# drtconway/zotmer

Hardware: AMD Instinct MI355X
Metric: Gk-mers/sec kmerize k=25 on synthetic 150bp FASTQ; achieved HBM GB/s fraction (higher is better)
Workload: dtype u64

## Files before the change

### zotmer_amd/csrc/context.hip

```cpp
#include <stdarg.h>
#include <string.h>

#include "internal.hpp"
#include <vector>

namespace zk {

int fail(zk_ctx* c, int code, const char* fmt, ...) {
    char buf[512];
    va_list ap;
    va_start(ap, fmt);
    vsnprintf(buf, sizeof buf, fmt, ap);
    va_end(ap);
    if (c) c->last_error = buf;
    return code;
}

void arena_reset(zk_ctx* c) { c->arena_off = 0; }

int arena_alloc(zk_ctx* c, uint64_t bytes, void** p) {
    const uint64_t need = (bytes + 255) & ~255ull;
    if (c->arena_off + need > c->arena_size) {
        if (c->arena_off != 0)
            return fail(c, ZK_ENOMEM, "workspace too small: %llu bytes in use, %llu more needed, %llu reserved (call zk_reserve)",
// ... 202 lines not shown
    if (c->status) (void)hipFree(c->status);
    if (c->part16) (void)hipFree(c->part16);
    if (c->d_ticket) (void)hipFree(c->d_ticket);
    if (c->d_xticket) (void)hipFree(c->d_xticket);
    if (c->d_err) (void)hipFree(c->d_err);
    if (c->d_scalars) (void)hipFree(c->d_scalars);
    if (c->h_scalars) (void)hipHostFree(c->h_scalars);
    if (c->own_stream && c->stream) (void)hipStreamDestroy(c->stream);
    delete c;
}

const char* zk_last_error(zk_ctx* c) { return c ? c->last_error.c_str() : g_create_error.c_str(); }

int zk_set_stream(zk_ctx* c, void* hip_stream) {
    if (!c) return ZK_EINVAL;
    enter(c);
    ZK_HIP(c, hipStreamSynchronize(c->stream));
    if (c->own_stream) { (void)hipStreamDestroy(c->stream); c->own_stream = false; }
    if (hip_stream) c->stream = (hipStream_t)hip_stream;
    else {
        ZK_HIP(c, hipStreamCreateWithFlags(&c->stream, hipStreamNonBlocking));
        c->own_stream = true;
    }
    return ZK_OK;
}

void* zk_get_stream(zk_ctx* c) { return c ? (void*)c->stream : nullptr; }

int zk_sync(zk_ctx* c) {
    if (!c) return ZK_EINVAL;
    enter(c);
    ZK_HIP(c, hipStreamSynchronize(c->stream));
    return ZK_OK;
}

int zk_reserve(zk_ctx* c, uint64_t workspace_bytes) {
    if (!c) return ZK_EINVAL;
    enter(c);
    if (workspace_bytes <= c->arena_size) return ZK_OK;
    arena_reset(c);
    void* p;
    ZK_TRY(arena_alloc(c, workspace_bytes, &p));
    arena_reset(c);
    return ZK_OK;
}

int zk_release_workspace(zk_ctx* c) {
    if (!c) return ZK_EINVAL;
    enter(c);
    ZK_HIP(c, hipStreamSynchronize(c->stream));
    if (c->arena) { ZK_HIP(c, hipFree(c->arena)); c->arena = nullptr; c->arena_size = 0; c->arena_off = 0; }
    if (c->aux) { ZK_HIP(c, hipFree(c->aux)); c->aux = nullptr; c->aux_size = 0; }
    if (c->status) { ZK_HIP(c, hipFree(c->status)); c->status = nullptr; c->status_words = 0; c->epoch = 0; }
    if (c->part16) { ZK_HIP(c, hipFree(c->part16)); c->part16 = nullptr; c->part16_words = 0; }
    return ZK_OK;
}

int zk_mem_info(zk_ctx* c, uint64_t* free_bytes, uint64_t* total_bytes) {
    if (!c) return ZK_EINVAL;
    enter(c);
    size_t f = 0, t = 0;
    ZK_HIP(c, hipMemGetInfo(&f, &t));
    if (free_bytes) *free_bytes = f;
    if (total_bytes) *total_bytes = t;
    return ZK_OK;
}

int zk_tune(zk_ctx* c, int what, int value) {
    if (!c) return ZK_EINVAL;
    enter(c);
    if (what == ZK_TUNE_SORT_VARIANT) { c->sort_variant = value; return ZK_OK; }
    if (what == ZK_TUNE_PAIRS_VARIANT) { c->pairs_variant = value; return ZK_OK; }
    if (what == ZK_TUNE_SHORT_SORT) { c->short_sort = value; return ZK_OK; }
    if (what == ZK_TUNE_SIDE_DIV) { c->side_div = value; return ZK_OK; }
    if (what == ZK_TUNE_WIDE_TILES) { c->wide_tiles = value ? 1 : 0; return ZK_OK; }
    if (what == ZK_TUNE_PACKED_PAIRS) { c->packed_pairs = value ? 1 : 0; return ZK_OK; }
    if (what == ZK_TUNE_EARLY_COLLAPSE) { c->early_collapse = value < 0 ? 0 : (value > 3 ? 3 : value); return ZK_OK; }
    if (what == ZK_TUNE_COMM_SELF_LOOP) { c->comm_self_loop = value ? 1 : 0; return ZK_OK; }
    if (what == ZK_TUNE_COMM_CHUNK) { c->comm_chunk_bytes = value > 0 ? (uint64_t)value : 0; return ZK_OK; }
    if (what == ZK_TUNE_STREAM_PASS) {
#ifdef ZK_PHASES
        c->stream_pass = value < 0 ? 0 : value;
#else
        if (value < 0 || value > 3) return fail(c, ZK_EINVAL, "stream pass variant %d (0, 1 or 3)", value);
        c->stream_pass = value;
#endif
        return ZK_OK;
    }
    if (what == ZK_TUNE_TAG_WORDS) { c->tag_words = value < 0 ? 0 : (value > 2 ? 2 : value); return ZK_OK; }
    if (what == ZK_TUNE_DEDUPE_VARIANT) { c->dedupe_variant = value < 0 ? -1 : (value & 3); return ZK_OK; }
    if (what == ZK_TUNE_KWAY) { c->kway = value < 0 ? 0 : (value > 2 ? 2 : value); return ZK_OK; }
    if (what == ZK_TUNE_TILE_SORT) { c->tile_sort = value ? 1 : 0; return ZK_OK; }
    if (what == ZK_TUNE_TAG_PASS) { c->tag_pass = value ? 1 : 0; return ZK_OK; }
    if (what == ZK_TUNE_DEDUPE_BITS) { c->dedupe_bits = value < 0 ? 0 : value; return ZK_OK; }
    if (what == ZK_TUNE_DEDUPE_LIMIT) { c->dedupe_limit = value < 1 ? 1 : (value > 65536 ? 65536 : value); return ZK_OK; }
    if (what == ZK_TUNE_STREAM_RANGES) { c->stream_ranges = value < 0 ? 0 : (value > 4096 ? 4096 : value); return ZK_OK; }
    if (what == ZK_TUNE_XCD_GROUP) {
        if (value < 0 || value > 32 || (value & (value - 1))) return fail(c, ZK_EINVAL, "xcd group must be 0 or a power of two <= 32");
        c->xcd_group = value;
        return ZK_OK;
    }
    return fail(c, ZK_EINVAL, "unknown tuning knob %d", what);
}

int zk_debug_buffer(zk_ctx* c, void* d_buf) {
    if (!c) return ZK_EINVAL;
    enter(c);
    c->dbg = (u64*)d_buf;
    return ZK_OK;
}

int zk_profile(zk_ctx* c, int enable) {
    if (!c) return ZK_EINVAL;
    enter(c);
    ZK_HIP(c, hipStreamSynchronize(c->stream));
    for (auto& r : c->prof) { (void)hipEventDestroy(r.a); (void)hipEventDestroy(r.b); }
    c->prof.clear();
    c->profile = enable != 0;
    return ZK_OK;
}

int zk_profile_read(zk_ctx* c, int tag, uint64_t* launches, double* total_ms, uint64_t* total_bytes) {
    if (!c) return ZK_EINVAL;
    enter(c);
    ZK_HIP(c, hipStreamSynchronize(c->stream));
    uint64_t n = 0, bytes = 0;
    double ms = 0;
    for (auto& r : c->prof) {
        if (r.tag != tag) continue;
        float t = 0;
        ZK_HIP(c, hipEventElapsedTime(&t, r.a, r.b));
        n++; ms += t; bytes += r.bytes;
    }
    if (launches) *launches = n;
    if (total_ms) *total_ms = ms;
    if (total_bytes) *total_bytes = bytes;
    return ZK_OK;
}

int zk_alloc(zk_ctx* c, uint64_t bytes, void** dptr) {
    if (!c || !dptr) return ZK_EINVAL;
    enter(c);
    *dptr = nullptr;
    if (bytes == 0) bytes = 256;
    hipError_t e = hipMalloc(dptr, bytes);
    if (e != hipSuccess) return fail(c, ZK_ENOMEM, "hipMalloc(%llu) failed: %s", (unsigned long long)bytes, hipGetErrorString(e));
    return ZK_OK;
}

int zk_free(zk_ctx* c, void* dptr) {
    if (!c) return ZK_EINVAL;
    enter(c);
    if (dptr) { ZK_HIP(c, hipStreamSynchronize(c->stream)); ZK_HIP(c, hipFree(dptr)); }
    return ZK_OK;
}

int zk_host_alloc(zk_ctx* c, uint64_t bytes, void** ptr) {
    if (!c || !ptr) return ZK_EINVAL;
    enter(c);
    *ptr = nullptr;
    hipError_t e = hipHostMalloc(ptr, bytes ? bytes : 256, hipHostMallocDefault);
    if (e != hipSuccess) return fail(c, ZK_ENOMEM, "hipHostMalloc(%llu) failed: %s", (unsigned long long)bytes, hipGetErrorString(e));
    return ZK_OK;
}

int zk_host_free(zk_ctx* c, void* ptr) {
    if (!c) return ZK_EINVAL;
// ... 41 lines not shown
```

### zotmer_amd/csrc/internal.hpp

```cpp
#pragma once
#include <hip/hip_runtime.h>
#include <stdint.h>
#include <stdio.h>
#include <string>
#include <vector>

#include "../../include/zotk.h"
#include "common.hpp"

struct zk_ctx {
    int device = 0;
    hipStream_t stream = nullptr;
    bool own_stream = false;
    int num_cus = 256;
    int sort_variant = 3;
    int short_sort = 0;
    int packed_pairs = 1;
    int wide_tiles = 1;
    int early_collapse = 1;
    int side_div = 8;
    int pairs_variant = 7;
    int stream_pass = 1;
    int tag_words = 2;
    int dedupe_variant = 0;
// ... 36 lines not shown

    void* ring = nullptr;

    struct ProfRec { int tag; uint64_t bytes; hipEvent_t a, b; };
    bool profile = false;
    std::vector<ProfRec> prof;
};

namespace zk {

int fail(zk_ctx* c, int code, const char* fmt, ...);
static inline void enter(zk_ctx* c) {
    int d = -1;
    if (c && (hipGetDevice(&d) != hipSuccess || d != c->device)) (void)hipSetDevice(c->device);
}
#define ZK_HIP(c, call)                                                                         \
    do {                                                                                        \
        hipError_t e__ = (call);                                                                \
        if (e__ != hipSuccess)                                                                  \
            return zk::fail((c), ZK_EHIP, "%s failed: %s (%s:%d)", #call, hipGetErrorString(e__), __FILE__, __LINE__); \
    } while (0)
#define ZK_TRY(expr)             \
    do {                         \
        int r__ = (expr);        \
        if (r__ != ZK_OK) return r__; \
    } while (0)

void arena_reset(zk_ctx* c);
int arena_alloc(zk_ctx* c, uint64_t bytes, void** p);
int arena_require(zk_ctx* c, uint64_t want, uint64_t must);
int aux_require(zk_ctx* c, uint64_t bytes, char** p);
int lookback_begin(zk_ctx* c, uint64_t words, uint32_t tiles, u32* epoch, u32* ticket_base);
int part16_begin(zk_ctx* c, uint64_t words, unsigned short** out);
int check_device_error(zk_ctx* c);

void prof_begin(zk_ctx* c, int tag, uint64_t algorithmic_bytes);
void prof_end(zk_ctx* c);
void prof_add_bytes(zk_ctx* c, int tag, uint64_t bytes);

static inline uint64_t div_up(uint64_t a, uint64_t b) { return (a + b - 1) / b; }

constexpr int MAX_PASSES = 8;
struct PassPlan {
    int passes;
    int shift[MAX_PASSES];
    int bits[MAX_PASSES];
};
int sort_workspace_bytes(uint64_t n, bool pairs, uint64_t* bytes);
int sort_keys(zk_ctx* c, u64* keys, u64* alt, uint64_t n, int key_bits, u64** result);
int sort_pairs(zk_ctx* c, u64* keys, u64* alt, u32* vals, u32* valt, uint64_t n, int key_bits, u64** rk, u32** rv);
int sort_keys_upper(zk_ctx* c, u64* keys, u64* alt, uint64_t n, int key_bits, int lo_bit, u64** result, int prof_tag = ZK_PROF_PASS_PACKED);
int sort_pairs_upper(zk_ctx* c, u64* keys, u64* alt, u32* vals, u32* valt, uint64_t n, int key_bits, int lo_bit, u64** rk, u32** rv);
int sort_pairs_mirrored(zk_ctx* c, const u64* src_k, const u32* src_v, u64* keys, u64* alt, u32* vals, u32* valt, uint64_t n, int K,
                        u64** rk, u32** rv, int lo_bit = 0);
int sort_pairs_rbits(zk_ctx* c);
struct StreamSample { int shift; uint64_t value; double max_ratio; uint64_t seen = 0, distinct = 0; bool want_distinct = false; };
struct StreamTags { bool written = false; u64* cuts = nullptr; uint32_t blocks = 0; };
struct StreamSrc { const u8* stream; uint64_t n_bytes; int K; int mode; int lo_bit; int hi_bit = 0; StreamSample* sample = nullptr;
                   StreamTags* tags = nullptr; };
int sort_rbits(zk_ctx* c);
PassPlan sort_plan_upper(zk_ctx* c, int key_bits, int lo_bit);
struct MirrorHist { int passes; int shift[4]; int bits[4]; u64* raw; };
int sort_first_bits(zk_ctx* c, int key_bits, int lo_bit);
struct DedupeResult {
    uint64_t n_out = 0;
    uint32_t flags = 0;
    uint32_t n_big = 0;
    u64 *cuts = nullptr, *nwords = nullptr, *incl = nullptr, *big = nullptr, *work = nullptr;
    u32* sub = nullptr;
    uint32_t chunks = 0;
    int pack = 0;
};
int dedupe_pass(zk_ctx* c, const u64* keys, uint64_t n, int key_bits, int b, int pack, u64* work, uint64_t cap, DedupeResult* r,
                uint64_t* n_in = nullptr, uint64_t max_chunks = 0, const u32* tags = nullptr, const u64* tag_cuts = nullptr);
int expand_tags(zk_ctx* c, const u32* tags, const u64* cuts, uint32_t blocks, int tag_bits, u64* keys_out, uint64_t first_block = 0, uint64_t n_blocks = 0);
int dedupe_finish(zk_ctx* c, const DedupeResult& r, u64* out_k, u32* out_c, u64* out_m = nullptr, int K = 0, int gbases = 0,
                  u64** mirror_hist = nullptr, int* mirror_group_bits = nullptr, bool packed_out = false);
int sort_keys_upper_counted(zk_ctx* c, u64* keys, u64* alt, uint64_t n, int key_bits, int lo_bit, u64* counted, u64** result);
int collapse_pass(zk_ctx* c, const u64* keys, uint64_t n, int shift, int bits, int pack, u64* out, uint64_t cap, uint64_t* n_out,
                  uint64_t max_tiles = 0);
int sort_stream(zk_ctx* c, const StreamSrc& src, u64* buf_a, u64* buf_b, uint64_t cap, uint64_t* n_keys,
                uint64_t acgt[4], u64** result);
struct StreamRows { u32* rows = nullptr; u64* offs = nullptr; u32 ranges = 0, radix = 0; u32* gcodes = nullptr; u16* gvalid = nullptr;
                    u32 strands = 1; };
int stream_hist(zk_ctx* c, const u8* stream, uint64_t n_bytes, int K, int mode, const PassPlan& plan, u64* ghist, u32 gstride,
                u64* d_acgt, u64* d_n, u64* rec_info, u64* sample, u32 sample_cap, int sample_shift, u64 sample_value, u32* sample_n,
                void* image_room, uint64_t image_room_bytes, StreamRows* out);
struct StreamPlanes { u16* dig; int shift, bits; };
int stream_pass0(zk_ctx* c, uint64_t n_bytes, int K, int mode, int shift, int bits, const u64* ghist0, const StreamRows& rows,
                 uint64_t first_nl, bool uniform, u64* kout, uint64_t n, int variant, const StreamPlanes* planes = nullptr);
int stream_pass1(zk_ctx* c, const u32* tags, const u16* dig, uint64_t n, const u64* ghist0, uint32_t radix0, int bits1, u32* tout, u64* cuts);
int tile_sort_top_bits(uint64_t n, int key_bits, int rbits);
int tile_sort(zk_ctx* c, u64* keys, u32* vals, uint64_t n, int key_bits, int top, bool* declined);
int tile_sort_count(zk_ctx* c, const u64* keys, uint64_t n, int key_bits, int top, u64* uniq, u32* counts, uint64_t cap, uint64_t* n_unique,
                    bool* declined);
int trim(zk_ctx* c, const u64* keys, const void* cnts, int cbits, uint64_t n, u64 lo, u64 hi, u64* ok, void* oc,
         uint64_t cap, uint64_t* n_out);
int project_dedupe(zk_ctx* c, const u64* keys, uint64_t n, int shift, u64* out, uint64_t cap, uint64_t* n_out);
int subsample(zk_ctx* c, const u64* keys, uint64_t n, u64 seed, double p, u64* out, uint64_t cap, uint64_t* n_out);
int sample_pairs(zk_ctx* c, const u64* keys, const u64* cnts, uint64_t n, u64 seed, double p, u64* ok, u64* oc, uint64_t cap,
                 uint64_t* n_out);
int subsample_pairs(zk_ctx* c, u64* keys, u32* cnts, uint64_t n, u64 seed, double p, uint64_t* n_out);
int encode_list(zk_ctx* c, const u8* stream, uint64_t n_bytes, int K, int both, u64* out, uint64_t cap, uint64_t* n_out,
                uint64_t acgt[4]);
int capture_filter(zk_ctx* c, const u8* stream, uint64_t n_bytes, int K, const u64* baits, uint64_t n_baits, u8* out,
                   uint64_t* n_reads, uint64_t* n_kept);
int rle_prefix(zk_ctx* c, const u64* sorted, uint64_t n, int pshift, u64* uniq, u32* counts, uint64_t cap, uint64_t* n_main,
               u64* side_k, u32* side_c, uint64_t side_cap, uint64_t* n_side);
int sample_heads(zk_ctx* c, const u64* keys, uint64_t n, uint64_t* sampled, uint64_t* heads);
int reduce_by_key(zk_ctx* c, const u64* sorted, const u32* w, uint64_t n, u64* uniq, u32* sums, uint64_t cap, uint64_t* n_out, int pack = 0,
                  uint64_t* max_sum = nullptr);
int rle(zk_ctx* c, const u64* sorted, uint64_t n, u64* uniq, u32* counts, uint64_t cap, uint64_t* n_unique, int pack = 0,
        bool* overflow = nullptr);
int count_hist(zk_ctx* c, const void* counts, int count_bits, uint64_t n, uint64_t* vals, uint64_t* freq,
               uint64_t cap_bins, uint64_t* n_bins);
int codec_decode(zk_ctx* c, const u64* d_words, uint64_t nw, int delta, u64* d_out, uint64_t cap, uint64_t* n_out);
int fastq_mask(zk_ctx* c, const u8* d_text, uint64_t n, uint32_t line_phase, u8* d_out, uint64_t* n_newlines);
int codec_encode(zk_ctx* c, const u64* d_vals, uint64_t n, int delta, u64* d_words, uint64_t cap, uint64_t* n_words);
int codec_encode_u32(zk_ctx* c, const u32* d_vals, uint64_t n, u64* d_words, uint64_t cap, uint64_t* n_words);
int scan64_inclusive(zk_ctx* c, u64* d_v, uint64_t n);
int add_u64(zk_ctx* c, u64* d_v, uint64_t n, u64 x);
void ring_destroy(zk_ctx* c);
int hash_partition(zk_ctx* c, const u64* keys, const void* cnts, int count_bits, uint64_t n, int world, u64 seed, u64* ok, void* oc,
                   uint64_t* offsets);
int checksum_any(zk_ctx* c, const u64* keys, const void* cnts, int count_bits, uint64_t n, uint64_t sums[3]);
int kway_union_sum(zk_ctx* c, int k, const u64* const* keys, const void* const* cnts, const uint64_t* ns, u64* out_k, void* out_c, int count_bits,
                   uint64_t cap, uint64_t* n_out, uint64_t acgt_w[4]);
int union_sum(zk_ctx* c, const u64* A, const void* cA, u64 nA, const u64* B, const void* cB, u64 nB, u64* ok, void* oc,
              int count_bits, uint64_t cap, uint64_t* n_out, uint64_t acgt_w[4], bool disjoint = false);
int union_sum_packed_b(zk_ctx* c, const u64* A, const u32* cA, u64 nA, const u64* Bp, u64 nB, int pack, u64* ok, u32* oc, uint64_t cap,
                       uint64_t* n_out, bool disjoint = false);
int union_sum_packed_ab(zk_ctx* c, const u64* Ap, u64 nA, const u64* Bp, u64 nB, int pack, u64* ok, u32* oc, uint64_t cap, uint64_t* n_out,
                        bool disjoint = false);
int column_sum(zk_ctx* c, const u64* rows, uint64_t n_rows, int cols, u64* out);
int project(zk_ctx* c, const u64* ref, u64 n_ref, const u64* B, const u64* cB, u64 nB, u64* ok, u64* oc, uint64_t cap, uint64_t* n_out);
int intersect_count(zk_ctx* c, const u64* A, u64 nA, const u64* B, u64 nB, uint64_t abc[3]);
}
```

### zotmer_amd/csrc/stream_pass.hip

```cpp
#include "internal.hpp"
#include "encode_tile.hpp"

#include <stdlib.h>
#include <type_traits>

namespace zk {

constexpr int P0_BLOCK = 512, P0_NW = 8, P0_TILE = P0_BLOCK * P0_NW, P0_IMG_WORDS = 320;
constexpr int SH_BLOCK = 512, SH_NW = 16, SH_TILE = SH_BLOCK * SH_NW;

struct StreamTiling {
    u32 rec;
    u32 rpt, cpr, wpr;
    u32 cpr_inv;
    u32 tile_bytes;
    u32 ranges;
    u64 range_bytes;
};

__host__ __device__ inline StreamTiling make_tiling(u64 n_bytes, u64 first_nl, int K, u32 ranges) {
    StreamTiling t = {};
    t.ranges = ranges ? ranges : 1;
    t.tile_bytes = P0_TILE;
    if (first_nl < 0x7fffffffull) {
        const u64 rec = first_nl + 1;
        const long long W = (long long)first_nl - K + 1;
        if (rec >= 16 && W >= 1 && n_bytes % rec == 0) {
            const u32 cpr = (u32)((W + P0_NW - 1) / P0_NW);
            u32 rpt = cpr <= (u32)P0_BLOCK ? ((u32)P0_BLOCK / cpr) / 16 * 16 : 0;
            const u32 fit = (u32)((16ull * (P0_IMG_WORDS - 3)) / rec) / 16 * 16;
            if (rpt > fit) rpt = fit;
            if (rpt >= 16 && (u64)rpt * rec * 50 > (u64)P0_TILE * 51) {
                t.rec = (u32)rec; t.rpt = rpt; t.cpr = cpr; t.wpr = (u32)W;
                t.cpr_inv = (u32)(((1ull << 32) + cpr - 1) / cpr);
                t.tile_bytes = rpt * (u32)rec;
            }
        }
    }
    const u64 tiles = (n_bytes + t.tile_bytes - 1) / t.tile_bytes;
    const u64 tpr = (tiles + t.ranges - 1) / t.ranges;
    t.range_bytes = (tpr ? tpr : 1) * (u64)t.tile_bytes;
    return t;
}

__device__ __forceinline__ void encode_swar16(const uint4 q, u32& codes, u32& vmask) {
    const u32 w[4] = {q.x, q.y, q.z, q.w};
    u32 cc = 0, vv = 0;
#pragma unroll
    for (int i = 0; i < 4; i++) {
        const u32 t = (w[i] >> 1) & 0x03030303u;
        const u32 code = t ^ ((t >> 1) & 0x01010101u);
        const u32 g = (code | (code >> 6) | (code >> 12) | (code >> 18)) & 0xffu;
        cc |= g << (8 * i);
        const u32 x = w[i] | 0x20202020u;
        const u32 t1 = (x >> 2) & ~(x >> 1);
        const u32 b4 = x >> 4;
        const u32 inner = (b4 & t1) | (~b4 & x & ~t1);
        const u32 ok = ~(x >> 7) & (x >> 6) & ~(x >> 3) & inner & 0x01010101u;
        const u32 n = (ok | (ok >> 7) | (ok >> 14) | (ok >> 21)) & 0xfu;
        vv |= n << (4 * i);
    }
    const u32 y = __brev(cc);
    codes = ((y >> 1) & 0x55555555u) | ((y & 0x55555555u) << 1);
    vmask = __brev(vv) >> 16;
}

__device__ __forceinline__ void shr128(u64 a, u64 b, u32 t, u32& w0, u32& w1, u32& w2) {
    const u32 s = t & 63u;
    const u64 lo_small = s ? ((b >> s) | (a << (64 - s))) : b;
    const u64 hi_small = a >> s;
    const bool big = t >= 64;
    const u64 lo = big ? hi_small : lo_small;
    const u64 hi = big ? 0ull : hi_small;
    w0 = (u32)lo; w1 = (u32)(lo >> 32); w2 = (u32)hi;
}

template <int NW>
struct WindowWords {
    u32 s0, s1, s2;
    u32 r0, r1, r2;
    __device__ __forceinline__ void init(u64 a, u64 b, u32 s, int K) {
        shr128(a, b, 128u - 2u * s - 2u * (NW - 1) - 2u * (u32)K, s0, s1, s2);
        const u64 rhi = rev_pairs(~b), rlo = rev_pairs(~a);
        shr128(rhi, rlo, 2u * s, r0, r1, r2);
    }
    __device__ __forceinline__ u32 xhi(int i) const { return __builtin_amdgcn_alignbit(s2, s1, 2 * (NW - 1 - i)); }
    __device__ __forceinline__ u32 xlo(int i) const { return __builtin_amdgcn_alignbit(s1, s0, 2 * (NW - 1 - i)); }
    __device__ __forceinline__ u32 bhi(int i) const { return __builtin_amdgcn_alignbit(r2, r1, 2 * i); }
    __device__ __forceinline__ u32 blo(int i) const { return __builtin_amdgcn_alignbit(r1, r0, 2 * i); }
};

__device__ __forceinline__ u64 runs_of_k(u64 v, int K) {
    int have = 1;
    while (2 * have <= K) { v &= v << have; have *= 2; }
    v &= v << (K - have);
    return v;
}

__device__ __forceinline__ u32 spread16(u32 x) {
    x = (x | (x << 8)) & 0x00FF00FFu;
    x = (x | (x << 4)) & 0x0F0F0F0Fu;
    x = (x | (x << 2)) & 0x33333333u;
    x = (x | (x << 1)) & 0x55555555u;
    return x;
}

struct SHistArgs {
    const u8* stream;
    u64 n_bytes;
    int K, mode;
    PassPlan plan;
    u32 binbase[MAX_PASSES];
    u32 nbins;
    u64* ghist;
    u32 gstride;
    u32* rows;
    u64* acgt;
    u64* rec_info;
    u64* sample;
    u32* sample_n;
    u32 sample_cap;
    int sample_shift;
    u64 sample_value;
    u32 revbase;
    u32 ranges, split;
    u32* gcodes;
    u16* gvalid;
    int dbg_atomics;
};

template <bool HI, bool TWO, int CANON_T = -1>
__global__ __launch_bounds__(SH_BLOCK, 4) void stream_hist_kernel(SHistArgs h) {
    extern __shared__ u32 bins[];
    __shared__ TileImage<SH_TILE> img;
    __shared__ u32 pshift[MAX_PASSES], pmask[MAX_PASSES], pbase[MAX_PASSES];
    const int tid = threadIdx.x;
    for (u32 i = tid; i < h.nbins; i += SH_BLOCK) bins[i] = 0;
    if (tid < MAX_PASSES) {
        pshift[tid] = (u32)h.plan.shift[tid] - (HI ? 32u : 0u);
        pmask[tid] = (1u << h.plan.bits[tid]) - 1u;
        pbase[tid] = h.binbase[tid];
    }
    const u64 first_nl = h.rec_info[0];
    const StreamTiling tl = make_tiling(h.n_bytes, first_nl, h.K, h.ranges);
    const u32 w = blockIdx.x / h.split, sp = blockIdx.x % h.split;
    const u64 B = (u64)w * tl.range_bytes;
    const u64 E = (B + tl.range_bytes < h.n_bytes) ? B + tl.range_bytes : h.n_bytes;
    const u32 ntile = B < E ? (u32)((E - B + SH_TILE - 1) / SH_TILE) : 0u;
    const int K = h.K;
    const int np = h.plan.passes;
    const u64 mask = ~0ull >> (64 - 2 * K);
    const u32 mlo = (u32)mask, mhi = (u32)(mask >> 32);
    const bool canon = CANON_T == 1 ? true : h.mode == ZK_KEYS_CANONICAL;
    const bool both = CANON_T != 1 && h.mode == ZK_KEYS_BOTH;
    const u32 sh0 = (u32)h.plan.shift[0] - (HI ? 32u : 0u), sh1 = (u32)h.plan.shift[1] - (HI ? 32u : 0u);
    const u32 dm0 = (1u << h.plan.bits[0]) - 1u, dm1 = (1u << h.plan.bits[1]) - 1u;
    const u32 base1 = h.binbase[1];
    const u32 nb0 = (u32)h.plan.bits[0], nb1 = (u32)h.plan.bits[1];
    const u32 ssh = (u32)h.sample_shift - (HI ? 32u : 0u);
    const typename std::conditional<HI, u32, u64>::type sval = (typename std::conditional<HI, u32, u64>::type)h.sample_value;
    u32 a0 = 0, a1 = 0, a2 = 0, a3 = 0, nl_count = 0, bad_count = 0;
    u32 rec = 0, m = 0, step_m = 0;
    if (first_nl < 0x7fffffffull) {
        rec = (u32)first_nl + 1u;
        m = (u32)((B + (u64)sp * SH_TILE + 16ull * tid) % rec);
        step_m = (u32)(((u64)h.split * SH_TILE) % rec);
    }
    uint4 q0 = make_uint4(0, 0, 0, 0), q1 = q0;
    auto issue = [&](u32 j) {
        const u64 P = B + (u64)j * SH_TILE;
        q0 = load_chunk16(h.stream, h.n_bytes, P + 16ull * tid);
        if (tid < 3) q1 = load_chunk16(h.stream, h.n_bytes, P + 16ull * (tid + SH_BLOCK));
    };
    if (sp < ntile) issue(sp);
    __syncthreads();
    for (u32 j = sp; j < ntile; j += h.split) {
        const u64 off = B + (u64)j * SH_TILE + 16ull * tid;
        const bool mine = off < E;
        {
            u32 cc, vv;
            encode_swar16(q0, cc, vv);
            if (rec) {
                if (mine) {
                    const int sep = (int)(rec - 1u) - (int)m;
                    const bool expect = sep >= 0 && sep < 16 && off + (u64)sep < h.n_bytes;
                    const u32 sepbit = expect ? (0x8000u >> (sep & 15)) : 0u;
                    if ((vv | sepbit) == 0xffffu) {
                        const u32 wsel = (sep & 12) == 0 ? q0.x : (sep & 12) == 4 ? q0.y : (sep & 12) == 8 ? q0.z : q0.w;
                        const bool isnl = ((wsel >> (8 * (sep & 3))) & 0xffu) == 0x0au;
                        nl_count += (expect && isnl) ? 1u : 0u;
                        bad_count += (expect && !isnl) ? 1u : 0u;
                    } else {
                        const u32 w4[4] = {q0.x, q0.y, q0.z, q0.w};
                        bool bad = false;
#pragma unroll
                        for (int q = 0; q < 4; q++) {
                            const u32 x = w4[q] ^ 0x0a0a0a0au;
                            const u32 t = ~(((x & 0x7f7f7f7fu) + 0x7f7f7f7fu) | x | 0x7f7f7f7fu);
                            nl_count += (u32)__popc(t);
                            const u32 want = (expect && (sep >> 2) == q) ? (0x80u << (8 * (sep & 3))) : 0u;
                            bad |= (t != want);
                        }
                        bad_count += bad ? 1u : 0u;
                    }
                }
                m += step_m;
                if (m >= rec) m -= rec;
            }
            img.codes[tid] = cc; img.valid[tid] = vv;
            if (mine && h.gcodes) { h.gcodes[off >> 4] = cc; h.gvalid[off >> 4] = (u16)vv; }
            if (tid < 3) {
                encode_swar16(q1, cc, vv);
                img.codes[tid + SH_BLOCK] = cc; img.valid[tid + SH_BLOCK] = vv;
            }
        }
        __syncthreads();
        if (j + h.split < ntile) issue(j + h.split);
        const u64 a = ((u64)img.codes[tid] << 32) | img.codes[tid + 1];
        const u64 b = ((u64)img.codes[tid + 2] << 32) | img.codes[tid + 3];
        u64 v = ((u64)img.valid[tid] << 48) | ((u64)img.valid[tid + 1] << 32) | ((u64)img.valid[tid + 2] << 16) | (u64)img.valid[tid + 3];
        v = runs_of_k(v, K);
        const u32 V16 = mine ? (u32)(v >> 48) : 0u;
        WindowWords<SH_NW> ww;
        ww.init(a, b, 0u, K);
        if (h.acgt) {
            const u32 Vs = spread16(V16);
            const u32 ff = (u32)(a >> 32);
// ... 379 lines not shown
            const u32 inc8 = wave_incl_scan_dpp(s8);
            const u32 before = wave ? (u32)__builtin_amdgcn_readlane((int)inc8, 8 * wave - 1) : 0u;
            tot = sm.cnt[tid];
            const u32 inc = wave_incl_scan_dpp(tot);
            O = before + inc - tot;
            u64 end = F + tot;
            if (end > Fend) { bad = 1; sm.anybad = 1; end = Fend > F ? Fend : F; }
            u64 Eo = last ? end : (end & ~(u64)(G - 1));
            if (Eo < F) Eo = F;
            flen = (u32)(Eo - F);
            head = (u32)(F & (G - 1)) ? G - (u32)(F & (G - 1)) : 0u;
            if (head > flen) head = flen;
            nu = (head ? 1u : 0u) + (flen - head + G - 1) / G;
            sm.nu[tid] = (u16)nu;
        }
        __syncthreads();
        {
            const uint4 c0 = reinterpret_cast<const uint4*>(sm.nu)[lane];
            const u32 s2 = c0.x + c0.y + c0.z + c0.w;
            const u32 s8 = (s2 & 0xffffu) + (s2 >> 16);
            const u32 inc8 = wave_incl_scan_dpp(s8);
            const u32 before = wave ? (u32)__builtin_amdgcn_readlane((int)inc8, 8 * wave - 1) : 0u;
            const u32 inc = wave_incl_scan_dpp(nu);
            u32 U = before + inc - nu;
            if (tid == 0) sm.nunits = (u32)__builtin_amdgcn_readlane((int)inc8, 63);
            sm.off[tid] = (u16)O;
            sm.cnt[tid] = tot - flen;
            sm.gbase[tid] = F - O;
            flen_dbg = flen;
            u32 slot = O, left = flen;
            if (head) { if (U < (u32)S::UNITS) sm.units[U] = unit_pack(slot, head, (u32)tid); U++; slot += head; left -= head; }
            while (left) {
                const u32 len = left < (u32)G ? left : (u32)G;
                if (U < (u32)S::UNITS) sm.units[U] = unit_pack(slot, len, (u32)tid);
                U++; slot += len; left -= len;
            }
            F += flen;
        }
        __syncthreads();
        P0_PHASE(2);
        {
            u32 at[NW];
#pragma unroll
            for (int i = 0; i < NW; i++) at[i] = sm.off[digit(key[i])];
#pragma unroll
            for (int i = 0; i < NW; i++) {
                const u32 slot = at[i] + rk[i];
                sm.exch[(((live >> i) & 1u) && slot < (u32)S::CAP) ? slot : (u32)S::CAP + (u32)lane] = key[i];
            }
#pragma unroll
            for (int j = 0; j < G - 1; j++) sm.exch[((u32)j < nck && O + j < (u32)S::CAP) ? O + j : (u32)S::CAP + (u32)lane] = ck[j];
            nck = tot - flen;
            ctail = O + flen;
        }
        P0_PHASE(3);
        __syncthreads();
        P0_PHASE(4);
        if (!last) {
            if ((u32)tid < nch) { sm.codes[tid] = qc; sm.valid[tid] = qv; }
            if (t + 2 < ntile) fetch(T0 + 2ull * tile_bytes);
        }
        P0_PHASE(5);
        }
        {
            const u32 nunits = (sm.anybad || sm.nunits > (u32)S::UNITS) ? 0u : sm.nunits;
            const u32 half = (PLANES || P0_MODE == 2 || !a.split_stores) ? nunits : (nunits / 2 + 127u) & ~127u;
            if constexpr (PLANES) store_units_planes(0, half < nunits ? half : nunits);
            else store_units(0, half < nunits ? half : nunits, std::integral_constant<int, 4>());
            held = half < nunits ? half : nunits; held_end = nunits;
        }
        P0_PHASE(6);
        __syncthreads();
        P0_PHASE(7);
    }
    if constexpr (!PLANES) { if (held < held_end) store_units(held, held_end, std::integral_constant<int, 2>()); }
    if (a.dbg && tid == 0) {
        for (int k = 0; k < 8; k++) a.dbg[(u64)w * 16 + k] = (u64)ph[k];
        a.dbg[(u64)w * 16 + 8] = ntile;
    }
    if (P0_MODE) return;
    if (bad || ((u32)tid < radix && (F != Fend || nck != 0))) atomicOr(a.err, ZK_DERR_MISMATCH);
}

int stream_ranges(zk_ctx* c) { return c->stream_ranges > 0 ? c->stream_ranges : 2 * (c->num_cus > 0 ? c->num_cus : 1); }

int stream_hist(zk_ctx* c, const u8* stream, uint64_t n_bytes, int K, int mode, const PassPlan& plan, u64* ghist, u32 gstride,
                u64* d_acgt, u64* d_n, u64* rec_info, u64* sample, u32 sample_cap, int sample_shift, u64 sample_value, u32* sample_n,
                void* image_room, uint64_t image_room_bytes, StreamRows* out) {
    SHistArgs h = {};
    h.stream = stream; h.n_bytes = n_bytes; h.K = K; h.mode = mode; h.plan = plan;
    u32 nb = 0;
    bool hi = 2 * K > 32;
    for (int p = 0; p < plan.passes; p++) { h.binbase[p] = nb; nb += 1u << plan.bits[p]; if (plan.shift[p] < 32) hi = false; }
    if (sample && sample_shift < 32) hi = false;
    const bool both = mode == ZK_KEYS_BOTH;
    const u32 strands = both ? 2u : 1u;
    h.revbase = nb;
    if (both) nb += 1u << plan.bits[0];
    h.nbins = nb;
    h.ghist = ghist; h.gstride = gstride;
    h.acgt = d_acgt; h.rec_info = rec_info;
    h.sample = sample; h.sample_n = sample_n; h.sample_cap = sample_cap; h.sample_shift = sample_shift; h.sample_value = sample_value;
    h.ranges = (u32)stream_ranges(c);
    h.split = 4;
    h.dbg_atomics = 2;
#ifdef ZK_PHASES
    if (const char* e = getenv("ZK_HIST_ATOMICS")) h.dbg_atomics = atoi(e);
#endif
    const u32 r0 = 1u << plan.bits[0];
    const uint64_t nchunks = (n_bytes + 15) / 16;
    u32* rows; u64* offs;
    ZK_TRY(arena_alloc(c, sizeof(u32) * (uint64_t)strands * h.ranges * r0, (void**)&rows));
    ZK_TRY(arena_alloc(c, sizeof(u64) * (uint64_t)strands * h.ranges * r0, (void**)&offs));
    const uint64_t codes_bytes = (sizeof(u32) * nchunks + 255) & ~255ull, image_bytes = codes_bytes + ((sizeof(u16) * nchunks + 255) & ~255ull);
    char* img = nullptr;
    if (image_room && image_room_bytes >= image_bytes + 256) img = (char*)(((uintptr_t)image_room + image_room_bytes - image_bytes) & ~(uintptr_t)255);
    else ZK_TRY(arena_alloc(c, image_bytes, (void**)&img));
    h.gcodes = (u32*)img; h.gvalid = (u16*)(img + codes_bytes);
    h.rows = rows;
    ZK_HIP(c, hipMemsetAsync(rows, 0, sizeof(u32) * (uint64_t)strands * h.ranges * r0, c->stream));
    ZK_HIP(c, hipMemsetAsync(ghist, 0, sizeof(u64) * MAX_PASSES * gstride, c->stream));
    if (d_acgt) ZK_HIP(c, hipMemsetAsync(d_acgt, 0, sizeof(u64) * 4, c->stream));
    const u32 grid = h.ranges * h.split;
    prof_begin(c, ZK_PROF_HIST_STREAM, n_bytes);
    const bool two = plan.passes == 2 && !both;
    if (hi && two && mode == ZK_KEYS_CANONICAL) hipLaunchKernelGGL((stream_hist_kernel<true, true, 1>), dim3(grid), dim3(SH_BLOCK), nb * sizeof(u32), c->stream, h);
    else if (hi && two) hipLaunchKernelGGL((stream_hist_kernel<true, true>), dim3(grid), dim3(SH_BLOCK), nb * sizeof(u32), c->stream, h);
    else if (hi) hipLaunchKernelGGL((stream_hist_kernel<true, false>), dim3(grid), dim3(SH_BLOCK), nb * sizeof(u32), c->stream, h);
    else if (two) hipLaunchKernelGGL((stream_hist_kernel<false, true>), dim3(grid), dim3(SH_BLOCK), nb * sizeof(u32), c->stream, h);
    else hipLaunchKernelGGL((stream_hist_kernel<false, false>), dim3(grid), dim3(SH_BLOCK), nb * sizeof(u32), c->stream, h);
    prof_end(c);
    ZK_HIP(c, hipGetLastError());
    out->rows = rows; out->offs = offs; out->ranges = h.ranges; out->strands = strands; out->radix = r0; out->gcodes = h.gcodes; out->gvalid = h.gvalid;
    return ZK_OK;
}

int stream_pass0(zk_ctx* c, uint64_t n_bytes, int K, int mode, int shift, int bits, const u64* ghist0, const StreamRows& rows,
                 uint64_t first_nl, bool uniform, u64* kout, uint64_t n, int variant, const StreamPlanes* planes) {
    if (bits < 1 || bits > 9 || (1u << bits) != rows.radix) return fail(c, ZK_EINTERNAL, "stream_pass0: %d digit bits, rows of %u", bits, rows.radix);
    if ((mode == ZK_KEYS_BOTH) != (rows.strands == 2)) return fail(c, ZK_EINTERNAL, "stream_pass0: rows of %u strands for mode %d", rows.strands, mode);
    const u32 grid = rows.ranges * rows.strands;
    hipLaunchKernelGGL(rows_scan_kernel, dim3((rows.radix + 255) / 256), dim3(256), 0, c->stream, rows.rows, ghist0, grid, rows.radix, rows.offs);
    P0Args a = {};
    a.gcodes = rows.gcodes; a.gvalid = rows.gvalid; a.n_bytes = n_bytes; a.K = K;
    a.tl = make_tiling(n_bytes, first_nl, K, rows.ranges);
    a.ranges = rows.ranges;
    a.by_record = (uniform && a.tl.rec) ? 1 : 0;
    a.shift = shift; a.bits = bits; a.offs = rows.offs; a.rows = rows.rows; a.kout = kout; a.n = n; a.err = c->d_err; a.dbg = c->dbg; a.dbg_mode = variant >> 8; a.split_stores = (variant & 0xff) == 3;
    const bool canon = mode == ZK_KEYS_CANONICAL, fast = 2 * K > 32 && shift >= 32;
    if (planes) {
        if (!canon || !fast) return fail(c, ZK_EINTERNAL, "stream_pass0: planes need the canonical fast plan");
        a.dig_out = planes->dig; a.dig_shift = planes->shift; a.dig_mask = (1u << planes->bits) - 1u;
        prof_begin(c, ZK_PROF_PASS_STREAM, n_bytes + 6 * n);
        hipLaunchKernelGGL((stream_pass0_kernel<9, 8, true, true, true>), dim3(rows.ranges), dim3(P0_BLOCK), 0, c->stream, a);
        prof_end(c);
        ZK_HIP(c, hipGetLastError());
        return ZK_OK;
    }
    prof_begin(c, ZK_PROF_PASS_STREAM, n_bytes + 8 * n);
    if (canon && fast) hipLaunchKernelGGL((stream_pass0_kernel<9, 8, true, true>), dim3(grid), dim3(P0_BLOCK), 0, c->stream, a);
    else if (canon) hipLaunchKernelGGL((stream_pass0_kernel<9, 8, true, false>), dim3(grid), dim3(P0_BLOCK), 0, c->stream, a);
    else if (fast) hipLaunchKernelGGL((stream_pass0_kernel<9, 8, false, true>), dim3(grid), dim3(P0_BLOCK), 0, c->stream, a);
    else hipLaunchKernelGGL((stream_pass0_kernel<9, 8, false, false>), dim3(grid), dim3(P0_BLOCK), 0, c->stream, a);
    prof_end(c);
    ZK_HIP(c, hipGetLastError());
    return ZK_OK;
}

}
```

Measured before the change: 145.4.

## Add 1024-thread wide stream pass0 kernel with half the ranges

Adds a 1024-thread variant of the stream pass-0 scatter kernel. In it, waves 0-7 own one radix digit each, and the other waves move carry keys at the same time. It is used by default when stream_pass is 1 and tag_pass is off. The tiling is parameterised by block geometry, and the stream ranges are halved to one per CU with the histogram split raised to 8. The intent is to double tile size per block and overlap carry movement with the scan, trading occupancy and LDS footprint for fewer, larger tiles.

New measurement: 154.4 (median of 6 runs). +6.2%, better.

```diff
diff --git a/zotmer_amd/csrc/context.hip b/zotmer_amd/csrc/context.hip
--- a/zotmer_amd/csrc/context.hip
+++ b/zotmer_amd/csrc/context.hip
@@ -308,7 +308,7 @@
 #ifdef ZK_PHASES
         c->stream_pass = value < 0 ? 0 : value;
 #else
-        if (value < 0 || value > 3) return fail(c, ZK_EINVAL, "stream pass variant %d (0, 1 or 3)", value);
+        if (value < 0 || value > 3) return fail(c, ZK_EINVAL, "stream pass variant %d (0, 1, 2 or 3)", value);
         c->stream_pass = value;
 #endif
         return ZK_OK;
diff --git a/zotmer_amd/csrc/internal.hpp b/zotmer_amd/csrc/internal.hpp
--- a/zotmer_amd/csrc/internal.hpp
+++ b/zotmer_amd/csrc/internal.hpp
@@ -142,7 +142,8 @@
 int sort_stream(zk_ctx* c, const StreamSrc& src, u64* buf_a, u64* buf_b, uint64_t cap, uint64_t* n_keys,
                 uint64_t acgt[4], u64** result);
 struct StreamRows { u32* rows = nullptr; u64* offs = nullptr; u32 ranges = 0, radix = 0; u32* gcodes = nullptr; u16* gvalid = nullptr;
-                    u32 strands = 1; };
+                    u32 strands = 1;
+                    bool wide = false; };
 int stream_hist(zk_ctx* c, const u8* stream, uint64_t n_bytes, int K, int mode, const PassPlan& plan, u64* ghist, u32 gstride,
                 u64* d_acgt, u64* d_n, u64* rec_info, u64* sample, u32 sample_cap, int sample_shift, u64 sample_value, u32* sample_n,
                 void* image_room, uint64_t image_room_bytes, StreamRows* out);
diff --git a/zotmer_amd/csrc/stream_pass.hip b/zotmer_amd/csrc/stream_pass.hip
--- a/zotmer_amd/csrc/stream_pass.hip
+++ b/zotmer_amd/csrc/stream_pass.hip
@@ -7,7 +7,11 @@
 namespace zk {
 
 constexpr int P0_BLOCK = 512, P0_NW = 8, P0_TILE = P0_BLOCK * P0_NW, P0_IMG_WORDS = 320;
+constexpr int PW_BLOCK = 1024, PW_NW = 8, PW_TILE = PW_BLOCK * PW_NW, PW_IMG_WORDS = 640;
 constexpr int SH_BLOCK = 512, SH_NW = 16, SH_TILE = SH_BLOCK * SH_NW;
+
+struct P0Geom { u32 block, nw, img_words; };
+__host__ __device__ constexpr P0Geom p0_geom(bool wide) { return wide ? P0Geom{PW_BLOCK, PW_NW, PW_IMG_WORDS} : P0Geom{P0_BLOCK, P0_NW, P0_IMG_WORDS}; }
 
 struct StreamTiling {
     u32 rec;
@@ -18,19 +22,20 @@
     u64 range_bytes;
 };
 
-__host__ __device__ inline StreamTiling make_tiling(u64 n_bytes, u64 first_nl, int K, u32 ranges) {
+__host__ __device__ inline StreamTiling make_tiling(u64 n_bytes, u64 first_nl, int K, u32 ranges, P0Geom g) {
     StreamTiling t = {};
+    const u32 tile = g.block * g.nw;
     t.ranges = ranges ? ranges : 1;
-    t.tile_bytes = P0_TILE;
+    t.tile_bytes = tile;
     if (first_nl < 0x7fffffffull) {
         const u64 rec = first_nl + 1;
         const long long W = (long long)first_nl - K + 1;
         if (rec >= 16 && W >= 1 && n_bytes % rec == 0) {
-            const u32 cpr = (u32)((W + P0_NW - 1) / P0_NW);
-            u32 rpt = cpr <= (u32)P0_BLOCK ? ((u32)P0_BLOCK / cpr) / 16 * 16 : 0;
-            const u32 fit = (u32)((16ull * (P0_IMG_WORDS - 3)) / rec) / 16 * 16;
+            const u32 cpr = (u32)((W + g.nw - 1) / g.nw);
+            u32 rpt = cpr <= g.block ? (g.block / cpr) / 16 * 16 : 0;
+            const u32 fit = (u32)((16ull * (g.img_words - 3)) / rec) / 16 * 16;
             if (rpt > fit) rpt = fit;
-            if (rpt >= 16 && (u64)rpt * rec * 50 > (u64)P0_TILE * 51) {
+            if (rpt >= 16 && (u64)rpt * rec * 50 > (u64)tile * 51) {
                 t.rec = (u32)rec; t.rpt = rpt; t.cpr = cpr; t.wpr = (u32)W;
                 t.cpr_inv = (u32)(((1ull << 32) + cpr - 1) / cpr);
                 t.tile_bytes = rpt * (u32)rec;
@@ -127,6 +132,7 @@
     u32* gcodes;
     u16* gvalid;
     int dbg_atomics;
+    P0Geom geom;
 };
 
 template <bool HI, bool TWO, int CANON_T = -1>
@@ -142,7 +148,7 @@
         pbase[tid] = h.binbase[tid];
     }
     const u64 first_nl = h.rec_info[0];
-    const StreamTiling tl = make_tiling(h.n_bytes, first_nl, h.K, h.ranges);
+    const StreamTiling tl = make_tiling(h.n_bytes, first_nl, h.K, h.ranges, h.geom);
     const u32 w = blockIdx.x / h.split, sp = blockIdx.x % h.split;
     const u64 B = (u64)w * tl.range_bytes;
     const u64 E = (B + tl.range_bytes < h.n_bytes) ? B + tl.range_bytes : h.n_bytes;
@@ -688,7 +694,271 @@
     if (bad || ((u32)tid < radix && (F != Fend || nck != 0))) atomicOr(a.err, ZK_DERR_MISMATCH);
 }
 
-int stream_ranges(zk_ctx* c) { return c->stream_ranges > 0 ? c->stream_ranges : 2 * (c->num_cus > 0 ? c->num_cus : 1); }
+template <int RBITS, int G>
+struct P0WideSmem {
+    static constexpr int RADIX = 1 << RBITS, CARRY = G - 1;
+    static constexpr int DEAD = PW_TILE, CB = PW_TILE + 64;
+    static constexpr int SLOTS = CB + RADIX * CARRY;
+    static constexpr int UNITS = (PW_TILE + RADIX * CARRY) / G + 2 * RADIX;
+    u64 exch[SLOTS];
+    u64 gbase[RADIX];
+    u32 units[UNITS];
+    u32 codes[PW_IMG_WORDS], valid[PW_IMG_WORDS];
+    alignas(16) u32 cnt[RADIX + 64];
+    u32 mv[RADIX];
+    u16 off[RADIX];
+    alignas(16) u16 nu[RADIX];
+    u32 nunits;
+    u32 anybad;
+};
+
+template <int RBITS, bool CANON, bool FAST>
+__global__ __launch_bounds__(PW_BLOCK) void stream_pass0_wide_kernel(P0Args a) {
+    constexpr int G = 16;
+    using S = P0WideSmem<RBITS, G>;
+    constexpr int RADIX = S::RADIX, NW = PW_NW, BLOCK = PW_BLOCK;
+    static_assert(2 * RADIX == BLOCK, "one digit per thread of waves 0-7");
+    static_assert(S::SLOTS < (1 << 14) && S::CARRY < 16 && RBITS <= 9, "unit words");
+    static_assert(sizeof(S) <= 160 * 1024, "LDS of a CU");
+    __shared__ S sm;
+    const int tid = threadIdx.x, lane = tid & 63, wave = __builtin_amdgcn_readfirstlane(tid >> 6);
+    const bool owner = wave < RADIX / 64;
+    const u32 w = blockIdx.x;
+    const bool rev = !CANON && w >= a.ranges;
+    const u32 radix = 1u << a.bits;
+    const u64 B = (u64)(rev ? w - a.ranges : w) * a.tl.range_bytes;
+    if (B >= a.n_bytes) return;
+    const u64 E = (B + a.tl.range_bytes < a.n_bytes) ? B + a.tl.range_bytes : a.n_bytes;
+    const u32 tile_bytes = a.by_record ? a.tl.tile_bytes : (u32)PW_TILE;
+    const u32 ntile = (u32)((E - B + tile_bytes - 1) / tile_bytes);
+    const u32 nch = tile_bytes / 16 + 3;
+    const int K = a.K;
+    const u64 mask = ~0ull >> (64 - 2 * K);
+    const u32 mlo = (u32)mask, mhi = (u32)(mask >> 32);
+    const u32 dmask = radix - 1u;
+    const u32 nchunks = (u32)((a.n_bytes + 15) >> 4);
+    auto digit = [&](u64 k) -> u32 {
+        if constexpr (FAST) return __builtin_amdgcn_ubfe((u32)(k >> 32), (u32)a.shift - 32u, (u32)a.bits);
+        else return (u32)(k >> a.shift) & dmask;
+    };
+    const bool mine = owner && (u32)tid < radix;
+    u64 F = mine ? a.offs[(u64)w * radix + tid] : 0ull;
+    const u64 Fend = F + (mine ? a.rows[(u64)w * radix + tid] : 0u);
+    u32 r = 0;
+    u32 bad = 0;
+    u32 flen_dbg = 0;
+    if (tid < RADIX + 64) sm.cnt[tid] = 0;
+    if (owner) sm.mv[tid] = 0;
+    if (tid == 0) { sm.anybad = 0; sm.units[0] = 0; }
+    u32 p0 = (u32)NW * tid, wlim = (1u << NW) - 1u;
+    if (a.by_record) {
+        const u32 rr = (u32)(((u64)tid * a.tl.cpr_inv) >> 32), j = tid - rr * a.tl.cpr;
+        p0 = rr * a.tl.rec + (u32)NW * j;
+        const int left = (int)a.tl.wpr - NW * (int)j;
+        wlim = (rr < a.tl.rpt) ? ((left >= NW) ? (1u << NW) - 1u : ((1u << (left > 0 ? left : 0)) - 1u)) : 0u;
+        if (rr >= a.tl.rpt) p0 = 0;
+    }
+    u32 qc = 0, qv = 0;
+    auto fetch = [&](u64 T) {
+        const u64 idx = (T >> 4) + (u32)tid;
+        const bool in = (u32)tid < nch && idx < nchunks;
+        qc = in ? a.gcodes[idx] : 0u;
+        qv = in ? (u32)a.gvalid[idx] : 0u;
+    };
+    fetch(B);
+    if ((u32)tid < nch) { sm.codes[tid] = qc; sm.valid[tid] = qv; }
+    if (ntile > 1) fetch(B + tile_bytes);
+    __syncthreads();
+    u32 ph[8] = {0, 0, 0, 0, 0, 0, 0, 0};
+    u32 tlast = a.dbg ? (u32)__builtin_amdgcn_s_memtime() : 0;
+    (void)tlast;
+    struct __attribute__((packed, aligned(8))) Key2 { u64 a, b; };
+    auto store_units = [&](u32 end) {
+        constexpr int NF = 2;
+        constexpr u32 LPU = G / 2, GROUPS = BLOCK / LPU;
+        const u32 j = 2u * ((u32)tid & (LPU - 1)), g0 = (u32)tid / LPU;
+        for (u32 base = 0; base < end; base += NF * GROUPS) {
+            u32 e4[NF];
+            u64 k4[NF], l4[NF], b4[NF];
+#pragma unroll
+            for (int g = 0; g < NF; g++) {
+                const u32 u = base + g * GROUPS + g0;
+                e4[g] = sm.units[u < end ? u : 0u];
+            }
+#pragma unroll
+            for (int g = 0; g < NF; g++) asm volatile("" : "+v"(e4[g]));
+#pragma unroll
+            for (int g = 0; g < NF; g++) {
+                const u32 d = (e4[g] >> 18) & (u32)(RADIX - 1), kc = e4[g] >> 27;
+                const u32 cs = (u32)S::CB + (u32)S::CARRY * d, ps = (e4[g] & 0x3fffu) - 16u;
+                k4[g] = sm.exch[j < kc ? cs + j : ps + j];
+                l4[g] = sm.exch[j + 1 < kc ? cs + j + 1 : ps + j + 1];
+                b4[g] = sm.gbase[d];
+            }
+#pragma unroll
+            for (int g = 0; g < NF; g++) asm volatile("" : "+v"(k4[g]), "+v"(l4[g]), "+v"(b4[g]));
+#pragma unroll
+            for (int g = 0; g < NF; g++) {
+                const u32 u = base + g * GROUPS + g0;
+                const u32 len1 = (e4[g] >> 14) & 15u;
+                u64* dst = a.kout + (b4[g] + (e4[g] & 0x3fffu) + j);
+                const bool fits = P0_MODE != 2 || b4[g] + (e4[g] & 0x3fffu) + G <= a.n;
+                if (u < end && P0_MODE != 1 && fits) {
+                    if (j < len1) { Key2 v; v.a = k4[g]; v.b = l4[g]; *reinterpret_cast<Key2*>(dst) = v; }
+                    else if (j == len1) *dst = k4[g];
+                }
+            }
+        }
+    };
+    for (u32 t = 0; t < ntile; t++) {
+        const u64 T0 = B + (u64)t * tile_bytes;
+        const bool last = t + 1 == ntile;
+        if (P0_MODE == 2 && t > 1) {
+            __syncthreads();
+            if (owner) sm.gbase[tid] += flen_dbg;
+            __syncthreads();
+        } else {
+        u64 key[NW];
+        u32 live;
+        {
+            const u32 j = p0 >> 4, s = p0 & 15u;
+            const u64 sa = ((u64)sm.codes[j] << 32) | sm.codes[j + 1];
+            const u64 sb = ((u64)sm.codes[j + 2] << 32) | sm.codes[j + 3];
+            u64 v = ((u64)sm.valid[j] << 48) | ((u64)sm.valid[j + 1] << 32) | ((u64)sm.valid[j + 2] << 16) | (u64)sm.valid[j + 3];
+            v = runs_of_k(v, K);
+            live = (__brev((u32)((v << s) >> (64 - NW))) >> (32 - NW)) & wlim;
+            if (T0 + p0 >= E) live = 0;
+            WindowWords<NW> ww;
+            ww.init(sa, sb, s, K);
+#pragma unroll
+            for (int i = 0; i < NW; i++) {
+                const u64 x = ((u64)(ww.xhi(i) & mhi) << 32) | (FAST ? ww.xlo(i) : (ww.xlo(i) & mlo));
+                const u64 xb = ((u64)(ww.bhi(i) & mhi) << 32) | (FAST ? ww.blo(i) : (ww.blo(i) & mlo));
+                if constexpr (CANON) key[i] = x < xb ? x : xb;
+                else key[i] = rev ? xb : x;
+            }
+        }
+        u32 rk[NW];
+#pragma unroll
+        for (int i = 0; i < NW; i++) rk[i] = atomicAdd(&sm.cnt[((live >> i) & 1u) ? digit(key[i]) : (u32)RADIX + (u32)lane], 1u);
+        P0_PHASE(0);
+        __syncthreads();
+        P0_PHASE(1);
+        u32 O = 0, tot = 0, flen = 0, head = 0, nu = 0, c = 0;
+        if (owner) {
+            const uint4 c0 = reinterpret_cast<const uint4*>(sm.cnt)[2 * lane], c1 = reinterpret_cast<const uint4*>(sm.cnt)[2 * lane + 1];
+            const u32 s8 = c0.x + c0.y + c0.z + c0.w + c1.x + c1.y + c1.z + c1.w;
+            const u32 inc8 = wave_incl_scan_dpp(s8);
+            const u32 before = wave ? (u32)__builtin_amdgcn_readlane((int)inc8, 8 * wave - 1) : 0u;
+            c = sm.cnt[tid];
+            const u32 inc = wave_incl_scan_dpp(c);
+            O = before + inc - c;
+            tot = r + c;
+            u64 end = F + tot;
+            if (end > Fend) { bad = 1; sm.anybad = 1; end = Fend > F ? Fend : F; }
+            u64 Eo = last ? end : (end & ~(u64)(G - 1));
+            if (Eo < F) Eo = F;
+            flen = (u32)(Eo - F);
+            head = (u32)(F & (G - 1)) ? G - (u32)(F & (G - 1)) : 0u;
+            if (head > flen) head = flen;
+            nu = (head ? 1u : 0u) + (flen - head + G - 1) / G;
+            sm.off[tid] = (u16)O;
+            sm.nu[tid] = (u16)nu;
+        } else {
+            const u32 q = (u32)tid - (u32)RADIX, j = 2u * (q & 7u);
+#pragma unroll
+            for (int h = 0; h < 2; h++) {
+                u32 m4[4], d4[4];
+                u64 v4[4], x4[4];
+#pragma unroll
+                for (int g = 0; g < 4; g++) { d4[g] = (u32)(4 * h + g) * (RADIX / 8) + (q >> 3); m4[g] = sm.mv[d4[g]]; }
+#pragma unroll
+                for (int g = 0; g < 4; g++) asm volatile("" : "+v"(m4[g]));
+#pragma unroll
+                for (int g = 0; g < 4; g++) {
+                    const u32 n = m4[g] >> 18, src = m4[g] & 0x3fffu;
+                    v4[g] = sm.exch[j < n ? src + j : (u32)S::DEAD + (u32)lane];
+                    x4[g] = sm.exch[j + 1 < n ? src + j + 1 : (u32)S::DEAD + (u32)lane];
+                }
+#pragma unroll
+                for (int g = 0; g < 4; g++) asm volatile("" : "+v"(v4[g]), "+v"(x4[g]));
+#pragma unroll
+                for (int g = 0; g < 4; g++) {
+                    const u32 n = m4[g] >> 18, dst = (u32)S::CB + (u32)S::CARRY * d4[g] + ((m4[g] >> 14) & 15u);
+                    sm.exch[j < n ? dst + j : (u32)S::DEAD + (u32)lane] = v4[g];
+                    sm.exch[j + 1 < n ? dst + j + 1 : (u32)S::DEAD + (u32)lane] = x4[g];
+                }
+            }
+        }
+        P0_PHASE(2);
+        __syncthreads();
+        P0_PHASE(3);
+        if (owner) {
+            const uint4 c0 = reinterpret_cast<const uint4*>(sm.nu)[lane];
+            const u32 s2 = c0.x + c0.y + c0.z + c0.w;
+            const u32 s8 = (s2 & 0xffffu) + (s2 >> 16);
+            const u32 inc8 = wave_incl_scan_dpp(s8);
+            const u32 before = wave ? (u32)__builtin_amdgcn_readlane((int)inc8, 8 * wave - 1) : 0u;
+            const u32 inc = wave_incl_scan_dpp(nu);
+            u32 U = before + inc - nu;
+            if (tid == 0) sm.nunits = (u32)__builtin_amdgcn_readlane((int)inc8, 63);
+            sm.gbase[tid] = F + r - O - 16u;
+            flen_dbg = flen;
+            const u32 ps = O + 16u - r;
+            u32 i = 0, left = flen;
+            if (head) {
+                const u32 kc = r < head ? r : head;
+                if (U < (u32)S::UNITS) sm.units[U] = unit_pack(ps + i, head, (u32)tid) | (kc << 27);
+                U++; i += head; left -= head;
+            }
+            while (left) {
+                const u32 len = left < (u32)G ? left : (u32)G;
+                const u32 kc = i < r ? (r - i < len ? r - i : len) : 0u;
+                if (U < (u32)S::UNITS) sm.units[U] = unit_pack(ps + i, len, (u32)tid) | (kc << 27);
+                U++; i += len; left -= len;
+            }
+            const u32 keep = tot - flen;
+            u32 src = O, dsto = r, n = c;
+            if (flen && flen >= r) { src = O + flen - r; dsto = 0; n = keep; }
+            if (dsto > (u32)S::CARRY) dsto = S::CARRY;
+            if (n > (u32)S::CARRY - dsto) n = (u32)S::CARRY - dsto;
+            sm.mv[tid] = src | (dsto << 14) | (n << 18);
+            r = keep < (u32)S::CARRY ? keep : (u32)S::CARRY;
+            sm.cnt[tid] = 0;
+            F += flen;
+        }
+        {
+            u32 at[NW];
+#pragma unroll
+            for (int i = 0; i < NW; i++) at[i] = sm.off[digit(key[i])];
+#pragma unroll
+            for (int i = 0; i < NW; i++) sm.exch[((live >> i) & 1u) ? at[i] + rk[i] : (u32)S::DEAD + (u32)lane] = key[i];
+        }
+        if (!last) {
+            if ((u32)tid < nch) { sm.codes[tid] = qc; sm.valid[tid] = qv; }
+            if (t + 2 < ntile) fetch(T0 + 2ull * tile_bytes);
+        }
+        P0_PHASE(4);
+        __syncthreads();
+        P0_PHASE(5);
+        }
+        {
+            const u32 nunits = (sm.anybad || sm.nunits > (u32)S::UNITS) ? 0u : sm.nunits;
+            store_units(nunits);
+        }
+        P0_PHASE(6);
+    }
+    if (a.dbg && tid == 0) {
+        for (int k = 0; k < 8; k++) a.dbg[(u64)w * 16 + k] = (u64)ph[k];
+        a.dbg[(u64)w * 16 + 8] = ntile;
+    }
+    if (P0_MODE) return;
+    if (bad || (mine && (F != Fend || r != 0))) atomicOr(a.err, ZK_DERR_MISMATCH);
+}
+
+static bool p0_wide(const zk_ctx* c) { return (c->stream_pass & 0xff) == 1 && !c->tag_pass; }
+
+int stream_ranges(zk_ctx* c, bool wide) { return c->stream_ranges > 0 ? c->stream_ranges : (wide ? 1 : 2) * (c->num_cus > 0 ? c->num_cus : 1); }
 
 int stream_hist(zk_ctx* c, const u8* stream, uint64_t n_bytes, int K, int mode, const PassPlan& plan, u64* ghist, u32 gstride,
                 u64* d_acgt, u64* d_n, u64* rec_info, u64* sample, u32 sample_cap, int sample_shift, u64 sample_value, u32* sample_n,
@@ -707,8 +977,10 @@
     h.ghist = ghist; h.gstride = gstride;
     h.acgt = d_acgt; h.rec_info = rec_info;
     h.sample = sample; h.sample_n = sample_n; h.sample_cap = sample_cap; h.sample_shift = sample_shift; h.sample_value = sample_value;
-    h.ranges = (u32)stream_ranges(c);
-    h.split = 4;
+    const bool wide = p0_wide(c);
+    h.geom = p0_geom(wide);
+    h.ranges = (u32)stream_ranges(c, wide);
+    h.split = wide ? 8 : 4;
     h.dbg_atomics = 2;
 #ifdef ZK_PHASES
     if (const char* e = getenv("ZK_HIST_ATOMICS")) h.dbg_atomics = atoi(e);
@@ -738,6 +1010,7 @@
     prof_end(c);
     ZK_HIP(c, hipGetLastError());
     out->rows = rows; out->offs = offs; out->ranges = h.ranges; out->strands = strands; out->radix = r0; out->gcodes = h.gcodes; out->gvalid = h.gvalid;
+    out->wide = wide;
     return ZK_OK;
 }
 
@@ -749,13 +1022,13 @@
     hipLaunchKernelGGL(rows_scan_kernel, dim3((rows.radix + 255) / 256), dim3(256), 0, c->stream, rows.rows, ghist0, grid, rows.radix, rows.offs);
     P0Args a = {};
     a.gcodes = rows.gcodes; a.gvalid = rows.gvalid; a.n_bytes = n_bytes; a.K = K;
-    a.tl = make_tiling(n_bytes, first_nl, K, rows.ranges);
+    a.tl = make_tiling(n_bytes, first_nl, K, rows.ranges, p0_geom(rows.wide));
     a.ranges = rows.ranges;
     a.by_record = (uniform && a.tl.rec) ? 1 : 0;
     a.shift = shift; a.bits = bits; a.offs = rows.offs; a.rows = rows.rows; a.kout = kout; a.n = n; a.err = c->d_err; a.dbg = c->dbg; a.dbg_mode = variant >> 8; a.split_stores = (variant & 0xff) == 3;
     const bool canon = mode == ZK_KEYS_CANONICAL, fast = 2 * K > 32 && shift >= 32;
     if (planes) {
-        if (!canon || !fast) return fail(c, ZK_EINTERNAL, "stream_pass0: planes need the canonical fast plan");
+        if (!canon || !fast || rows.wide) return fail(c, ZK_EINTERNAL, "stream_pass0: planes need the canonical fast plan and the 512-thread kernel");
         a.dig_out = planes->dig; a.dig_shift = planes->shift; a.dig_mask = (1u << planes->bits) - 1u;
         prof_begin(c, ZK_PROF_PASS_STREAM, n_bytes + 6 * n);
         hipLaunchKernelGGL((stream_pass0_kernel<9, 8, true, true, true>), dim3(rows.ranges), dim3(P0_BLOCK), 0, c->stream, a);
@@ -764,7 +1037,12 @@
         return ZK_OK;
     }
     prof_begin(c, ZK_PROF_PASS_STREAM, n_bytes + 8 * n);
-    if (canon && fast) hipLaunchKernelGGL((stream_pass0_kernel<9, 8, true, true>), dim3(grid), dim3(P0_BLOCK), 0, c->stream, a);
+    if (rows.wide) {
+        if (canon && fast) hipLaunchKernelGGL((stream_pass0_wide_kernel<9, true, true>), dim3(grid), dim3(PW_BLOCK), 0, c->stream, a);
+        else if (canon) hipLaunchKernelGGL((stream_pass0_wide_kernel<9, true, false>), dim3(grid), dim3(PW_BLOCK), 0, c->stream, a);
+        else if (fast) hipLaunchKernelGGL((stream_pass0_wide_kernel<9, false, true>), dim3(grid), dim3(PW_BLOCK), 0, c->stream, a);
+        else hipLaunchKernelGGL((stream_pass0_wide_kernel<9, false, false>), dim3(grid), dim3(PW_BLOCK), 0, c->stream, a);
+    } else if (canon && fast) hipLaunchKernelGGL((stream_pass0_kernel<9, 8, true, true>), dim3(grid), dim3(P0_BLOCK), 0, c->stream, a);
     else if (canon) hipLaunchKernelGGL((stream_pass0_kernel<9, 8, true, false>), dim3(grid), dim3(P0_BLOCK), 0, c->stream, a);
     else if (fast) hipLaunchKernelGGL((stream_pass0_kernel<9, 8, false, true>), dim3(grid), dim3(P0_BLOCK), 0, c->stream, a);
     else hipLaunchKernelGGL((stream_pass0_kernel<9, 8, false, false>), dim3(grid), dim3(P0_BLOCK), 0, c->stream, a);
```
